# LoganWilliams1/mhm2_kmer_analysis_v2

Measured on AMD Instinct MI355X. Metric: k-mers/sec (kcount stage) at k=21, higher is better.
Workload: dtype u64

## Files before the change

mhm2_kmer_analysis_v2_amd/csrc/kc_bucketed.hpp:

```cpp
#pragma once
#include "kc_kernels.hpp"

namespace kc {

constexpr int WGB = 1024;
constexpr int SUPER_SPAN = 16 * WGB - PRE - POST;
using TileSuper = TileGeo<WGB, SUPER_SPAN>;
static_assert(TileSuper::GPT == 1 && TileSuper::NGROUP == WGB, "one group per thread");
constexpr int PMAX = 1024;
constexpr int GMAX = 512;

template <int NL> struct Rnd {
  static constexpr int RPOS = NL == 1 ? 16 : NL == 2 ? 8 : 4;
  static constexpr int RPOS_READS = NL == 1 ? 8 : NL <= 3 ? 4 : 2;
  static constexpr size_t STAGE = ((size_t)WGB * RPOS + 64) * NL * 8;
  static constexpr size_t STAGE_READS = ((size_t)WGB * RPOS_READS + 64) * NL * 8;
};

struct Geom {
  uint32_t G, P1, P2, S;
  uint32_t log2CH1, log2CH2;
  uint32_t L1MAX, L2MAX;
  uint32_t A1;
  uint32_t A2;
  uint32_t cp;
  uint32_t la, lb;
  uint32_t k2;
  uint32_t own_lo, own_hi;
  uint32_t rec6;
};

struct BucketBufs {
  uint64_t *rec1;
  uint32_t *chain1;
  uint32_t *cnt1;
  uint32_t *used1;
  uint64_t *rec2;
  uint32_t *chain2;
  uint32_t *cnt2;
  uint32_t *base2;
  uint32_t *flag;
  uint64_t *ovf1;
  uint64_t *ovf2;
  uint64_t ovf1_cap, ovf2_cap;
  uint32_t *done1;
  uint32_t *used2;
};

constexpr uint32_t FLAT_MAX = 256;
struct FlatSrc {
  const uint32_t *cnt;
  const uint64_t *at;
  uint32_t F, nbo;
  uint32_t b_lo, b_hi;
};

enum {
  CB_OVF1 = 0, CB_OVF2, CB_FATAL, CB_FLAGGED_RECS, CB_DUMP, CB_ENTRIES, CB_OUT_RESERVED, CB_COUNT = 16
};
enum { FATAL_OVF1 = 1,
       FATAL_ARENA2 = 2,
       FATAL_OVF2 = 4 };


__device__ __forceinline__ uint32_t hash_b1(uint64_t h, const Geom &g) { return (((uint32_t)h & 0xFFFFu) * g.P1) >> 16; }
__device__ __forceinline__ uint32_t hash_b2(uint64_t h, const Geom &g) { return ((((uint32_t)h >> 16) & 0xFFFFu) * g.P2) >> 16; }
__device__ __forceinline__ uint32_t hash_slot(uint64_t h, uint32_t S) {
  return (uint32_t)(h >> 32) & (S - 1u);
}

__device__ __forceinline__ uint64_t cp_mix_rec(uint64_t keyrec, const Geom &g) {
  const uint32_t sh = 64u - g.k2;
  return (kc_feistel_fwd(keyrec >> sh, (int)(g.k2 >> 1)) << sh) | (keyrec & KC_EXT_MASK);
}
__device__ __forceinline__ uint64_t cp_unmix_rec(uint64_t mixrec, const Geom &g) {
  const uint32_t sh = 64u - g.k2;
  return (kc_feistel_inv(mixrec >> sh, (int)(g.k2 >> 1)) << sh) | (mixrec & KC_EXT_MASK);
}
__device__ __forceinline__ uint32_t cp_b1(uint64_t rec, const Geom &g) { return (uint32_t)(rec >> (64u - g.la)); }
__device__ __forceinline__ uint32_t cp_b2(uint64_t rec, const Geom &g) { return (uint32_t)(rec >> (64u - g.la - g.lb)) & (g.P2 - 1u); }
__device__ __forceinline__ uint32_t cp_pack32(uint64_t rec, const Geom &g) {
  const uint32_t rb = g.k2 - g.la - g.lb;
  return (((uint32_t)(rec >> (64u - g.k2)) & ((1u << rb) - 1u)) << 6) | ((uint32_t)rec & (uint32_t)KC_EXT_MASK);
}
__device__ __forceinline__ uint64_t cp_unpack_rec(uint32_t rec32, size_t region, const Geom &g) {
  const uint32_t rb = g.k2 - g.la - g.lb;
  const uint64_t mix = ((uint64_t)region << rb) | (uint64_t)(rec32 >> 6);
  return (kc_feistel_inv(mix, (int)(g.k2 >> 1)) << (64u - g.k2)) | (uint64_t)(rec32 & (uint32_t)KC_EXT_MASK);
}

template <int NL>
__device__ __forceinline__ uint64_t rec_hash(const uint64_t (&rec)[NL]) {
  uint64_t key[NL];
#pragma unroll
  for (int j = 0; j < NL; j++) key[j] = rec[j];
  key[NL - 1] &= ~KC_EXT_MASK;
  return kc_hash<NL>(key);
}

__device__ __forceinline__ void lds_barrier() { asm volatile("s_waitcnt lgkmcnt(0)\n\ts_barrier" ::: "memory"); }

__device__ __forceinline__ int fresh_tid() {
  int t = threadIdx.x;
  asm volatile("" : "+v"(t));
  return t;
}

struct ScanLDS {
  uint32_t wsum[32];
  uint32_t total;
};

__device__ __forceinline__ uint32_t wave_incl_scan(uint32_t v) {
  v += (uint32_t)__builtin_amdgcn_update_dpp(0, (int)v, 0x111, 0xF, 0xF, false);
  v += (uint32_t)__builtin_amdgcn_update_dpp(0, (int)v, 0x112, 0xF, 0xF, false);
  v += (uint32_t)__builtin_amdgcn_update_dpp(0, (int)v, 0x114, 0xF, 0xF, false);
  v += (uint32_t)__builtin_amdgcn_update_dpp(0, (int)v, 0x118, 0xF, 0xF, false);
  v += (uint32_t)__builtin_amdgcn_update_dpp(0, (int)v, 0x142, 0xA, 0xF, false);
  v += (uint32_t)__builtin_amdgcn_update_dpp(0, (int)v, 0x143, 0xC, 0xF, false);
  return v;
}

__device__ __forceinline__ uint32_t block_excl_scan(uint32_t v, ScanLDS &S) {
  static_assert(WGB / 64 <= 16, "the wave totals must fit one row of 16 lanes");
  const int tid = threadIdx.x;
  const int wave = __builtin_amdgcn_readfirstlane(tid >> 6);
  const uint32_t incl = wave_incl_scan(v);
  if (lane_id() == 63) S.wsum[wave] = incl;
  lds_barrier();
  const uint32_t w = (lane_id() < WGB / 64) ? S.wsum[lane_id()] : 0u;
  uint32_t wi = w;
  wi += (uint32_t)__builtin_amdgcn_update_dpp(0, (int)wi, 0x111, 0xF, 0xF, false);
  wi += (uint32_t)__builtin_amdgcn_update_dpp(0, (int)wi, 0x112, 0xF, 0xF, false);
  wi += (uint32_t)__builtin_amdgcn_update_dpp(0, (int)wi, 0x114, 0xF, 0xF, false);
  wi += (uint32_t)__builtin_amdgcn_update_dpp(0, (int)wi, 0x118, 0xF, 0xF, false);
  const uint32_t wave_pre = (uint32_t)__builtin_amdgcn_readlane((int)(wi - w), wave);
  const uint32_t total = (uint32_t)__builtin_amdgcn_readlane((int)wi, WGB / 64 - 1);
  if (tid == 0) S.total = total;
  return incl - v + wave_pre;
}

struct SplitLDS {
  uint32_t hist[2][PMAX + 64];
  uint4 dst[PMAX];
  uint32_t arena_used;
  uint32_t arena_top;
  ScanLDS scan;
};

__device__ __forceinline__ uint32_t hist_rank(SplitLDS &L, int buf, uint32_t b, bool valid) {
  return atomicAdd(&L.hist[buf][valid ? b : (uint32_t)PMAX + lane_id()], 1u);
}

#ifdef KC_STAMPS
#define KC_SPLIT_STAMP(k)                                                                 \
  if (threadIdx.x == 0 && D.stamps) {                                                     \
    const unsigned long long tn_ = __builtin_amdgcn_s_memtime();                          \
    atomicAdd((unsigned long long *)&D.stamps[k], tn_ - *D.tprev);                        \
    *D.tprev = tn_;                                                                       \
  }
#else
#define KC_SPLIT_STAMP(k)
#endif

struct ChainDest {
#ifdef KC_STAMPS
  uint64_t *stamps;
  unsigned long long *tprev;
#endif
  uint64_t *arena;
  uint32_t *chain;
  uint32_t log2CH, LMAX;
  uint32_t arena_cap;
  uint32_t arena_base;
  uint32_t own_lo, own_hi;
};

struct ChainState {
  uint32_t cur;
  uint32_t last;
};

struct RunPlace {
  uint32_t x, y, fit, w;
};
__device__ __forceinline__ RunPlace split_reserve(SplitLDS &L, uint32_t tid, uint32_t v, uint32_t excl, const ChainDest &D, ChainState &st) {
  const uint32_t CHm = (1u << D.log2CH) - 1u;
  const uint32_t base = st.cur;
  uint32_t fit = v;
  const uint64_t room = ((uint64_t)D.LMAX << D.log2CH) - base;
  if ((uint64_t)fit > room) fit = (uint32_t)room;
  const uint32_t have = (base + CHm) >> D.log2CH;
  uint32_t k = ((base + fit + CHm) >> D.log2CH) - have, a = 0;
  if (k) {
    const bool own = tid >= D.own_lo && tid < D.own_hi;
    if (own) {
      a = atomicAdd(&L.arena_used, k);
      const uint32_t left = D.arena_cap - min(D.arena_cap, L.arena_top);
      if (a + k > left) {
        k = a < left ? left - a : 0;
        const uint64_t cap = ((uint64_t)(have + k) << D.log2CH) - base;
        if ((uint64_t)fit > cap) fit = (uint32_t)cap;
      }
    } else {
      const uint32_t t = atomicAdd(&L.arena_top, k);
      const uint32_t left = D.arena_cap - min(D.arena_cap, L.arena_used);
      if (t + k > left) {
        k = 0;
        const uint64_t cap = ((uint64_t)have << D.log2CH) - base;
        if ((uint64_t)fit > cap) fit = (uint32_t)cap;
      } else {
        a = D.arena_cap - t - k;
      }
    }
    uint32_t *ch = D.chain + (size_t)tid * D.LMAX + have;
    for (uint32_t i = 0; i < k; i++) ch[i] = D.arena_base + a + i;
  }
  RunPlace q;
  q.x = ((st.last - D.arena_base - (base >> D.log2CH)) << D.log2CH) + base - excl;
  q.y = ((a - have) << D.log2CH) + base - excl;
  q.fit = fit;
  q.w = (base & CHm) ? min(fit, (CHm + 1u) - (base & CHm)) : 0u;
  if (k) st.last = D.arena_base + a + k - 1;
  st.cur = base + fit;
  return q;
}

template <int NL, int R, int RS = 10, class RecFn>
__device__ __forceinline__ uint32_t split_stage(SplitLDS &L, uint64_t *sorted, uint16_t *sbucket, int buf, uint32_t P, RecFn rec_of,
                                                const uint32_t (&br)[R], const ChainDest &D, ChainState &st) {
  static_assert(R * WGB <= 32768, "positions in the staging must fit 16 bits");
  static_assert(RS == 10 || R * WGB <= 65536, "ranks must fit the bits above RS");
  const int tid = fresh_tid();
  KC_SPLIT_STAMP(1)
  const uint32_t v = ((uint32_t)tid < P) ? L.hist[buf][tid] : 0u;
  const uint32_t excl = block_excl_scan(v, L.scan);
  if ((uint32_t)tid < P) {
    const RunPlace q = split_reserve(L, (uint32_t)tid, v, excl, D, st);
    L.dst[tid] = make_uint4(q.x, q.y, excl | (q.fit << 16), q.w);
    L.hist[buf][tid] = excl;
    L.hist[buf ^ 1][tid] = 0;
  }
  lds_barrier();
  KC_SPLIT_STAMP(2)
  const uint32_t total = L.scan.total;
  constexpr int H = R < 8 ? R : 8;
#pragma unroll
  for (int j0 = 0; j0 < R; j0 += H) {
    uint32_t pos[H];
#pragma unroll
    for (int j = 0; j < H; j++) pos[j] = L.hist[buf][br[j0 + j] & (PMAX - 1)];
#pragma unroll
    for (int j = 0; j < H; j++) {
      const uint32_t bj = br[j0 + j];
      const uint32_t p = bj != ~0u ? pos[j] + (bj >> RS) : (uint32_t)(R * WGB) + lane_id();
      uint64_t r[NL];
      rec_of(j0 + j, r);
#pragma unroll
      for (int w = 0; w < NL; w++) sorted[(size_t)p * NL + w] = r[w];
      if (sbucket) sbucket[p] = (uint16_t)(bj & (PMAX - 1));
    }
  }
  lds_barrier();
  KC_SPLIT_STAMP(3)
  return total;
}

template <int NL, class BucketFn, class OvfFn, class StoreFn>
__device__ __forceinline__ void split_copy_out(SplitLDS &L, const uint64_t *sorted, const uint16_t *sbucket, uint32_t total, const ChainDest &D,
                                               BucketFn bucket_of, OvfFn overflow, StoreFn store) {
  const int tid = fresh_tid();
  constexpr int U = NL == 1 ? 4 : 2;
  const size_t arena0 = (size_t)D.arena_base << D.log2CH;
  for (uint32_t i0 = tid; i0 < total; i0 += U * WGB) {
    uint64_t r[U][NL];
    uint32_t b[U];
    uint4 d[U];
#pragma unroll
    for (int u = 0; u < U; u++) {
      const uint32_t i = i0 + u * WGB;
      const uint32_t ii = i < total ? i : i0;
#pragma unroll
      for (int w = 0; w < NL; w++) r[u][w] = sorted[(size_t)ii * NL + w];
      if (sbucket) b[u] = sbucket[ii];
    }
    if (!sbucket) {
#pragma unroll
      for (int u = 0; u < U; u++) b[u] = bucket_of(r[u]);
    }
#pragma unroll
    for (int u = 0; u < U; u++) d[u] = L.dst[b[u]];
    bool spill = false;
#pragma unroll
    for (int u = 0; u < U; u++) {
      const uint32_t i = i0 + u * WGB;
      const uint32_t j = i - (d[u].z & 0xFFFFu);
      const bool live = i < total, fits = j < (d[u].z >> 16);
      const uint32_t at = (j < d[u].w ? d[u].x : d[u].y) + i;
      if (live && fits) store(arena0 + at, r[u]);
      spill |= live && !fits;
    }
    if (__any(spill)) {
#pragma unroll
      for (int u = 0; u < U; u++) {
        const uint32_t i = i0 + u * WGB;
        if (i < total && i - (d[u].z & 0xFFFFu) >= (d[u].z >> 16)) overflow(b[u], r[u]);
      }
    }
  }
  KC_SPLIT_STAMP(4)
}

template <int NL>
__device__ __forceinline__ void store_words(uint64_t *arena, size_t i, const uint64_t (&r)[NL]) {
#pragma unroll
  for (int w = 0; w < NL; w++) arena[i * NL + w] = r[w];
}

__device__ __forceinline__ ChainState split_load_state(SplitLDS &L, uint32_t P, const uint32_t *cnt, const uint32_t *chain,
                                                       uint32_t LMAX, uint32_t log2CH, uint32_t used, uint32_t top = 0) {
  const int tid = threadIdx.x;
  ChainState st;
  st.cur = 0;
  st.last = 0;
  if ((uint32_t)tid < P) {
    const uint32_t c = cnt ? cnt[tid] : 0u;
    st.cur = c;
    if (c & ((1u << log2CH) - 1u)) st.last = chain[(size_t)tid * LMAX + (c >> log2CH)];
    L.hist[0][tid] = 0;
    L.hist[1][tid] = 0;
  }
  if (tid == 0) {
    L.arena_used = used;
    L.arena_top = top;
  }
  return st;
}

__global__ __launch_bounds__(WGB) void kc_arena_probe_kernel(uint64_t *arena, size_t words_per_wg, uint32_t rounds) {
  uint64_t *mine = arena + (size_t)blockIdx.x * words_per_wg;
  const uint32_t t = threadIdx.x, b = t >> 3, w = t & 7u;
  const size_t chunks = words_per_wg / 512u;
  const size_t hop = chunks > 1024u ? (chunks - 1024u) / 31u : 0u;
  for (uint32_t r = 0; r < rounds; r++) {
    const size_t first = (size_t)((r >> 3) & 31u) * hop;
#pragma unroll
    for (uint32_t j = 0; j < 8; j++) {
      const size_t chunk = first + b + 128u * j;
      const size_t at = chunk * 512u + (size_t)(r & 7u) * 8u + w;
      if (at < words_per_wg) mine[at] = (uint64_t)r;
    }
  }
}

struct L1LDS {
  TileLDS<TileSuper> tile;
  SplitLDS sp;
};

template <int NL>
__device__ __forceinline__ ChainDest l1_dest(const Geom &gm, const BucketBufs &bb, uint32_t g) {
  ChainDest D;
#ifdef KC_STAMPS
  D.stamps = nullptr;
  D.tprev = nullptr;
#endif
  D.arena = bb.rec1 + (((size_t)g * gm.A1) << gm.log2CH1) * NL;
  D.chain = bb.chain1 + (size_t)g * gm.P1 * gm.L1MAX;
  D.log2CH = gm.log2CH1;
  D.LMAX = gm.L1MAX;
  D.arena_cap = gm.A1;
  D.arena_base = 0;
  D.own_lo = gm.own_lo;
  D.own_hi = gm.own_hi;
  return D;
}

__device__ __forceinline__ ChainDest l1_dest6(const Geom &gm, const BucketBufs &bb, uint32_t g) {
  ChainDest D = l1_dest<1>(gm, bb, g);
  D.arena = reinterpret_cast<uint64_t *>(reinterpret_cast<uint8_t *>(bb.rec1) + (((size_t)g * gm.A1) << gm.log2CH1) * 6);
  return D;
}

template <int NL, bool CP>
__device__ __forceinline__ void l1_overflow(const Geom &gm, const BucketBufs &bb, uint64_t *cb, const uint64_t (&r)[NL]) {
  const uint64_t o = atomicAdd((unsigned long long *)&cb[CB_OVF1], 1ULL);
  if (o < bb.ovf1_cap) {
#pragma unroll
    for (int w = 0; w < NL; w++) bb.ovf1[o * NL + w] = (CP && w == 0) ? cp_unmix_rec(r[w], gm) : r[w];
  } else {
    atomicOr((unsigned long long *)&cb[CB_FATAL], (unsigned long long)FATAL_OVF1);
  }
}

template <int KT, int RPOS, bool SH, class TL>
__device__ __forceinline__ void cp_run_fixed(const TL &L, int lp0, bool active, const Geom &gm, const ExtractArgs &a, uint32_t (&lo)[RPOS],
                                             uint32_t (&bk)[RPOS]) {
  const int K = KT ? KT : (int)a.k;
  const int NB = RPOS + K + 1;
  static_assert(RPOS + KT + 1 <= 32 && RPOS % 8 == 0 && PRE % 8 == 0, "the window must fit one word and never start word-aligned");
  const uint64_t *W = reinterpret_cast<const uint64_t *>(L.codes);
  const uint32_t *OK = reinterpret_cast<const uint32_t *>(L.ok);
  const int p = lp0 - 1, q = p >> 5, s = p & 31;
  const uint64_t w0 = W[q], w1 = W[q + 1];
  const uint32_t ok0 = OK[q], ok1 = OK[q + 1], g0 = L.gap[q], g1 = L.gap[q + 1];
  const uint64_t Wn = (w0 << (2 * s)) | (w1 >> (64 - 2 * s));
  const uint32_t nok = ~__builtin_amdgcn_alignbit(ok1, ok0, (uint32_t)s);
  const uint32_t gapw = __builtin_amdgcn_alignbit(g1, g0, (uint32_t)s);
  const uint64_t Rn = kc_rc_word(Wn) << (64 - 2 * NB);
  const uint64_t MID = ((1ULL << (2 * K)) - 1ULL) << 2;
  const uint32_t MK = (1u << K) - 1u;
#pragma unroll
  for (int j = 0; j < RPOS; j++) {
    const uint64_t x = Wn >> (64 - 2 * (j + K + 2)), y = Rn >> (64 - 2 * (RPOS - 1 - j + K + 2));
    const uint64_t CMP = (K & 1) ? (MID | 3ULL) : MID;
    const bool swap = (y & CMP) < (x & CMP);
    const uint64_t sel = swap ? y : x;
    const uint32_t na = (nok >> j) & 1u, nb = (nok >> (j + K + 1)) & 1u;
    const uint32_t le = ((uint32_t)(sel >> (2 * K + 2)) & 3u) | ((swap ? nb : na) << 2);
    const uint32_t re = ((uint32_t)sel & 3u) | ((swap ? na : nb) << 2);
    uint32_t Lh = (uint32_t)(sel >> (K + 2)) & MK, Rh = (uint32_t)(sel >> 2) & MK;
    bool valid = active && ((gapw >> (j + 1)) & ((1u << (K + 1)) - 1u)) == 0u;
    if (SH) {
      uint64_t key[1] = {(((uint64_t)Lh << K) | Rh) << (64 - 2 * K)};
      const uint32_t owner = a.reference_owner ? 0u : kc_owner_of_hash(kc_hash<1>(key), a.rank_n);
      if (a.reference_owner) {
        uint64_t rk[1];
        kc_revcomp<1>(key, K, rk);
        valid = valid && kc_reference_owner<1>(key, rk, K, a.rank_n) == a.rank_me;
      } else {
        valid = valid && owner == a.rank_me;
      }
    }
    Lh ^= kc_feistel_f(Rh, 0, K);
    Rh ^= kc_feistel_f(Lh, 1, K);
    Lh ^= kc_feistel_f(Rh, 2, K);
    const uint64_t mix = ((uint64_t)Lh << K) | Rh;
    lo[j] = (uint32_t)mix;
    bk[j] = valid ? ((uint32_t)(mix >> (2 * K - gm.la)) | (le << 10) | (re << 13)) : ~0u;
  }
}

template <int K, int RPOS, class TL>
__device__ __forceinline__ uint32_t cut_run_fixed(const TL &L, int lp0, bool active, uint64_t (&rec)[RPOS], uint64_t (&h)[RPOS]) {
  constexpr int NB = RPOS + K + 1;
  static_assert(NB <= 32 && RPOS % 8 == 0 && PRE % 8 == 0, "the window must fit one word and never start word-aligned");
  const uint64_t *W = reinterpret_cast<const uint64_t *>(L.codes);
  const uint32_t *OK = reinterpret_cast<const uint32_t *>(L.ok);
  const int p = lp0 - 1, q = p >> 5, s = p & 31;
  const uint64_t w0 = W[q], w1 = W[q + 1];
  const uint32_t ok0 = OK[q], ok1 = OK[q + 1], g0 = L.gap[q], g1 = L.gap[q + 1];
  const uint64_t Wn = (w0 << (2 * s)) | (w1 >> (64 - 2 * s));
  const uint32_t nok = ~__builtin_amdgcn_alignbit(ok1, ok0, (uint32_t)s);
  const uint32_t gapw = __builtin_amdgcn_alignbit(g1, g0, (uint32_t)s);
  const uint64_t Rn = kc_rc_word(Wn) << (64 - 2 * NB);
  constexpr uint64_t MID = ((1ULL << (2 * K)) - 1ULL) << 2;
  constexpr uint64_t CMP = (K & 1) ? (MID | 3ULL) : MID;
  uint32_t okm = 0;
#pragma unroll
  for (int j = 0; j < RPOS; j++) {
    const uint64_t x = Wn >> (64 - 2 * (j + K + 2)), y = Rn >> (64 - 2 * (RPOS - 1 - j + K + 2));
    const bool swap = (y & CMP) < (x & CMP);
    const uint64_t sel = swap ? y : x;
    const uint32_t na = (nok >> j) & 1u, nb = (nok >> (j + K + 1)) & 1u;
    const uint32_t le = ((uint32_t)(sel >> (2 * K + 2)) & 3u) | ((swap ? nb : na) << 2);
    const uint32_t re = ((uint32_t)sel & 3u) | ((swap ? na : nb) << 2);
    const uint64_t key = (sel >> 2) << (64 - 2 * K);
    const uint64_t kk[1] = {key};
    h[j] = kc_hash<1>(kk);
    rec[j] = key | (uint64_t)((le & 4u) ? 4u : le) | ((uint64_t)((re & 4u) ? 4u : re) << 3);
    const bool valid = active && ((gapw >> (j + 1)) & ((1u << (K + 1)) - 1u)) == 0u;
    okm |= valid ? (1u << j) : 0u;
  }
  return okm;
}

template <int NL, int FMT, bool CP, bool SH>
__global__ __launch_bounds__(WGB) void kc_l1_reads_kernel(ExtractArgs a, Geom gm, BucketBufs bb, uint64_t nsuper, uint32_t rot,
                                                          uint64_t *ctrs, uint64_t *cb) {
  extern __shared__ __align__(16) uint8_t smem[];
  L1LDS &L = *reinterpret_cast<L1LDS *>(smem);
  uint64_t *sorted = reinterpret_cast<uint64_t *>(smem + ((sizeof(L1LDS) + 15) & ~size_t(15)));
  uint16_t *sbucket = CP ? nullptr : reinterpret_cast<uint16_t *>(smem + ((sizeof(L1LDS) + 15) & ~size_t(15)) + Rnd<NL>::STAGE_READS);
  constexpr int RPOS = Rnd<NL>::RPOS_READS;
  const int tid = threadIdx.x;
  const uint32_t g = (blockIdx.x + rot) % gm.G, P1 = gm.P1;
  ChainDest D = l1_dest<NL>(gm, bb, g);
#ifdef KC_STAMPS
  unsigned long long tprev_ = __builtin_amdgcn_s_memtime();
  D.stamps = cb + 8;
  D.tprev = &tprev_;
#endif
  ChainState cst = split_load_state(L.sp, P1, bb.cnt1 + (size_t)g * P1, D.chain, D.LMAX, D.log2CH, bb.used1[g], bb.used1[gm.G + g]);
  __syncthreads();
  uint32_t n_ins = 0;
  int buf = 0;
  TileRaw<TileSuper> raw;
  auto first_of = [&](uint64_t st) -> uint64_t { return (FMT != FMT_SEQBLOCK && st < nsuper) ? a.tile_first[st] : 0; };
  tile_prefetch<FMT, TileSuper>(raw, a, a.pos0 + (int64_t)blockIdx.x * SUPER_SPAN, tid, first_of(blockIdx.x), blockIdx.x < nsuper);
  uint64_t next_first = first_of((uint64_t)blockIdx.x + gridDim.x);
  constexpr int RUNS = SUPER_SPAN / RPOS;
  static_assert(SUPER_SPAN % RPOS == 0, "runs must tile the span");
  constexpr int NROUND = (RUNS + WGB - 1) / WGB;
  for (int64_t it = -1;; it++) {
    const uint64_t st = (uint64_t)blockIdx.x + (uint64_t)(it < 0 ? 0 : it) * gridDim.x;
    const bool work = it >= 0;
    if (work && st >= nsuper) break;
#pragma unroll 1
    for (int round = 0; round < NROUND; round++) {
      uint64_t rec[RPOS][NL];
      uint32_t br[RPOS];
      uint32_t total = 0;
      if (work) {
      const int run_id = round * WGB + tid;
      const bool active = run_id < RUNS;
      const int lp0 = PRE + (active ? run_id : 0) * RPOS;
      KmerRun<NL> run;
      run_begin<NL>(run, L.tile, lp0, a.k);
#pragma unroll
      for (int j = 0; j < RPOS; j++) {
        uint64_t h = 0;
        uint32_t owner = 0;
        bool valid = run_kmer<NL, !CP>(run, j, lp0, a.k, rec[j], h, SH ? a.rank_n : 1u, SH ? a.reference_owner : 0u, SH ? &owner : nullptr) && active;
        if (SH) {
          if (CP && !a.reference_owner) {
            uint64_t key[NL];
#pragma unroll
            for (int w = 0; w < NL; w++) key[w] = rec[j][w];
            key[NL - 1] &= ~KC_EXT_MASK;
            owner = kc_owner_of_hash(kc_hash<NL>(key), a.rank_n);
          }
          valid = valid && owner == a.rank_me;
        }
        if (CP) rec[j][0] = cp_mix_rec(rec[j][0], gm);
        br[j] = valid ? (CP ? cp_b1(rec[j][0], gm) : hash_b1(h, gm)) : ~0u;
        if (j + 1 < RPOS) run_advance<NL>(run, j, lp0, a.k);
      }
#pragma unroll
      for (int j = 0; j < RPOS; j++) {
        const bool valid = br[j] != ~0u;
        const uint32_t rank = hist_rank(L.sp, buf, br[j] & (PMAX - 1), valid);
        br[j] = valid ? (br[j] | (rank << 10)) : ~0u;
        n_ins += valid ? 1u : 0u;
      }
      KC_SPLIT_STAMP(0)
      lds_barrier();
      total = split_stage<NL, RPOS>(
          L.sp, sorted, sbucket, buf, P1,
          [&](int j, uint64_t (&o)[NL]) {
#pragma unroll
            for (int w = 0; w < NL; w++) o[w] = rec[j][w];
          },
          br, D, cst);
      }
      if (round == NROUND - 1) {
        const uint64_t nst = work ? st + gridDim.x : st;
        tile_encode<FMT, TileSuper>(L.tile, raw, a, a.pos0 + (int64_t)nst * SUPER_SPAN, ctrs, tid, nst < nsuper);
        tile_prefetch<FMT, TileSuper>(raw, a, a.pos0 + (int64_t)(nst + gridDim.x) * SUPER_SPAN, tid, next_first, nst + gridDim.x < nsuper);
        next_first = first_of(nst + 2 * (uint64_t)gridDim.x);
        KC_SPLIT_STAMP(5)
      }
      if (work) {
        split_copy_out<NL>(
            L.sp, sorted, sbucket, total, D, [&](const uint64_t (&r)[NL]) { return cp_b1(r[0], gm); },
            [&](uint32_t, const uint64_t (&r)[NL]) { l1_overflow<NL, CP>(gm, bb, cb, r); },
            [&](size_t i, const uint64_t (&r)[NL]) { store_words<NL>(D.arena, i, r); });
        buf ^= 1;
      }
    }
  }
  if ((uint32_t)tid < P1) bb.cnt1[(size_t)g * P1 + tid] = cst.cur;
  if (tid == 0) {
    bb.used1[g] = min(L.sp.arena_used, gm.A1);
    bb.used1[gm.G + g] = min(L.sp.arena_top, gm.A1);
  }
  for (int o = 32; o > 0; o >>= 1) n_ins += __shfl_down(n_ins, o);
  if (lane_id() == 0 && n_ins) atomicAdd((unsigned long long *)&ctrs[CTR_INSERTED], (unsigned long long)n_ins);
}

constexpr int R16 = 16;
constexpr uint32_t ST16_MAIN = (uint32_t)WGB * R16 + PMAX;
constexpr uint32_t ST16_SLOTS = ST16_MAIN + 64;
static_assert(SUPER_SPAN % R16 == 0 && SUPER_SPAN / R16 <= WGB, "one run of sixteen positions per thread covers the super-tile");
static_assert(ST16_MAIN < 65536, "staging positions fit 16 bits");
constexpr size_t l1x16_lds_bytes() { return ((sizeof(L1LDS) + 15) & ~size_t(15)) + (size_t)ST16_SLOTS * 6; }

template <class MidFn>
__device__ __forceinline__ uint32_t split_stage_pairs(SplitLDS &L, uint32_t *slo, uint16_t *sbk, int buf, uint32_t P, const uint32_t (&lo)[R16],
                                                      const uint32_t (&br)[R16], const ChainDest &D, ChainState &st, MidFn mid) {
  const int tid = fresh_tid();
  KC_SPLIT_STAMP(1)
  const uint32_t v = ((uint32_t)tid < P) ? L.hist[buf][tid] : 0u;
  const uint32_t excl = block_excl_scan((v + 1u) & ~1u, L.scan);
// ... 31 lines not shown
    }
    uint4 d;
    d.x = ((st.last - D.arena_base - (base >> D.log2CH)) << D.log2CH) + base - excl;
    d.y = ((a - have) << D.log2CH) + base - excl;
    d.z = excl | (v << 16);
    d.w = fit | (((base & CHm) ? min(fit, (CHm + 1u) - (base & CHm)) : 0u) << 16);
    L.dst[tid] = d;
    if (k) st.last = D.arena_base + a + k - 1;
    st.cur = base + fit;
    L.hist[buf][tid] = excl;
    L.hist[buf ^ 1][tid] = 0;
  }
  lds_barrier();
  KC_SPLIT_STAMP(2)
  const uint32_t total = L.scan.total;
#pragma unroll
  for (int j0 = 0; j0 < R16; j0 += 8) {
    uint32_t pos[8];
#pragma unroll
    for (int j = 0; j < 8; j++) pos[j] = L.hist[buf][br[j0 + j] & (PMAX - 1)];
#pragma unroll
    for (int j = 0; j < 8; j++) {
      const uint32_t bj = br[j0 + j];
      const uint32_t p = bj != ~0u ? pos[j] + (bj >> 16) : ST16_MAIN + lane_id();
      slo[p] = lo[j0 + j];
      sbk[p] = (uint16_t)bj;
    }
  }
  mid();
  lds_barrier();
  KC_SPLIT_STAMP(3)
  return total;
}

struct __attribute__((packed, aligned(2))) Rec6Pair {
  uint32_t w0, w1, w2;
};
struct __attribute__((packed, aligned(2))) Rec6 {
  uint32_t lo;
  uint16_t bk;
};
static_assert(sizeof(Rec6Pair) == 12 && sizeof(Rec6) == 6, "six bytes a record");

template <class OvfFn>
__device__ __forceinline__ void split_copy_out_pairs(SplitLDS &L, const uint32_t *slo, const uint16_t *sbk, uint32_t total, const ChainDest &D,
                                                     const Geom &gm, OvfFn overflow) {
  const int tid = fresh_tid();
  constexpr int U = 2;
  uint8_t *const arena0 = reinterpret_cast<uint8_t *>(D.arena) + ((size_t)D.arena_base << D.log2CH) * 6;
  const uint32_t shb = 64u - gm.la, shl = 64u - gm.k2;
  for (uint32_t i0 = 2u * (uint32_t)tid; i0 < total; i0 += 2u * U * WGB) {
    uint64_t lo2[U];
    uint32_t bk2[U];
    uint4 d[U];
#pragma unroll
    for (int u = 0; u < U; u++) {
      const uint32_t i = i0 + 2u * (uint32_t)u * WGB;
      const uint32_t ii = i < total ? i : i0;
      lo2[u] = *reinterpret_cast<const uint64_t *>(slo + ii);
      bk2[u] = *reinterpret_cast<const uint32_t *>(sbk + ii);
    }
#pragma unroll
    for (int u = 0; u < U; u++) d[u] = L.dst[bk2[u] & (PMAX - 1)];
    bool odd = false;
#pragma unroll
    for (int u = 0; u < U; u++) {
      const uint32_t i = i0 + 2u * (uint32_t)u * WGB;
      const uint32_t j = i - (d[u].z & 0xFFFFu), v = d[u].z >> 16, fit = d[u].w & 0xFFFFu, wold = d[u].w >> 16;
      const bool live = i < total;
      const bool f0 = live && j < fit, real1 = live && j + 1u < v, f1 = real1 && j + 1u < fit;
      const uint32_t at0 = (j < wold ? d[u].x : d[u].y) + i, at1 = (j + 1u < wold ? d[u].x : d[u].y) + i + 1u;
      const bool pair = f0 && f1 && at1 == at0 + 1u;
      if (pair) {
        const uint32_t l1 = (uint32_t)(lo2[u] >> 32);
        Rec6Pair r;
        r.w0 = (uint32_t)lo2[u];
        r.w1 = (bk2[u] & 0xFFFFu) | (l1 << 16);
        r.w2 = (l1 >> 16) | (bk2[u] & 0xFFFF0000u);
        *reinterpret_cast<Rec6Pair *>(arena0 + (size_t)at0 * 6) = r;
      } else if (f0) {
        Rec6 r;
        r.lo = (uint32_t)lo2[u];
        r.bk = (uint16_t)bk2[u];
        *reinterpret_cast<Rec6 *>(arena0 + (size_t)at0 * 6) = r;
      }
      odd |= (real1 && !pair) || (live && !f0);
    }
    if (__any(odd)) {
#pragma unroll
      for (int u = 0; u < U; u++) {
        const uint32_t i = i0 + 2u * (uint32_t)u * WGB;
        if (i >= total) continue;
        const uint32_t j = i - (d[u].z & 0xFFFFu), v = d[u].z >> 16, fit = d[u].w & 0xFFFFu, wold = d[u].w >> 16;
        const uint32_t at0 = (j < wold ? d[u].x : d[u].y) + i, at1 = (j + 1u < wold ? d[u].x : d[u].y) + i + 1u;
        const uint32_t l0 = (uint32_t)lo2[u], l1 = (uint32_t)(lo2[u] >> 32);
        const uint64_t bh = (uint64_t)(bk2[u] & (PMAX - 1)) << shb;
        const uint64_t ra = bh | ((uint64_t)l0 << shl) | (uint64_t)((bk2[u] >> 10) & 63u);
        const uint64_t rb = bh | ((uint64_t)l1 << shl) | (uint64_t)(bk2[u] >> 26);
        const bool f0 = j < fit, real1 = j + 1u < v, f1 = real1 && j + 1u < fit;
        if (!f0) overflow(ra);
        if (real1 && !(f0 && f1 && at1 == at0 + 1u)) {
          if (f1) {
            Rec6 r;
            r.lo = l1;
            r.bk = (uint16_t)(bk2[u] >> 16);
            *reinterpret_cast<Rec6 *>(arena0 + (size_t)at1 * 6) = r;
          } else {
            overflow(rb);
          }
        }
      }
    }
  }
  KC_SPLIT_STAMP(4)
}

template <int FMT, bool SH, int KK>
__global__ __launch_bounds__(WGB) void kc_l1_reads16_kernel(ExtractArgs a, Geom gm, BucketBufs bb, uint64_t nsuper, uint32_t rot, uint64_t *ctrs,
                                                            uint64_t *cb) {
  extern __shared__ __align__(16) uint8_t smem[];
  L1LDS &L = *reinterpret_cast<L1LDS *>(smem);
  uint32_t *slo = reinterpret_cast<uint32_t *>(smem + ((sizeof(L1LDS) + 15) & ~size_t(15)));
  uint16_t *sbk = reinterpret_cast<uint16_t *>(slo + ST16_SLOTS);
  const int tid = threadIdx.x;
  const uint32_t g = (blockIdx.x + rot) % gm.G, P1 = gm.P1;
  ChainDest D = l1_dest6(gm, bb, g);
#ifdef KC_STAMPS
  unsigned long long tprev_ = __builtin_amdgcn_s_memtime();
  D.stamps = cb + 8;
  D.tprev = &tprev_;
#endif
  ChainState cst = split_load_state(L.sp, P1, bb.cnt1 + (size_t)g * P1, D.chain, D.LMAX, D.log2CH, bb.used1[g], bb.used1[gm.G + g]);
  __syncthreads();
  uint32_t n_ins = 0;
  int buf = 0;
  TileRaw<TileSuper> raw;
  auto first_of = [&](uint64_t st) -> uint64_t { return (FMT != FMT_SEQBLOCK && st < nsuper) ? a.tile_first[st] : 0; };
  tile_prefetch<FMT, TileSuper>(raw, a, a.pos0 + (int64_t)blockIdx.x * SUPER_SPAN, tid, first_of(blockIdx.x), blockIdx.x < nsuper);
  uint64_t next_first = first_of((uint64_t)blockIdx.x + gridDim.x);
  constexpr int RUNS = SUPER_SPAN / R16;
  {
    const int ft = fresh_tid();
    tile_encode<FMT, TileSuper>(L.tile, raw, a, a.pos0 + (int64_t)blockIdx.x * SUPER_SPAN, ctrs, ft, blockIdx.x < nsuper);
    tile_prefetch<FMT, TileSuper>(raw, a, a.pos0 + (int64_t)((uint64_t)blockIdx.x + gridDim.x) * SUPER_SPAN, ft, next_first,
                                  (uint64_t)blockIdx.x + gridDim.x < nsuper);
    next_first = first_of((uint64_t)blockIdx.x + 2 * (uint64_t)gridDim.x);
  }
  for (uint64_t st = blockIdx.x; st < nsuper; st += gridDim.x) {
    uint32_t lo[R16], br[R16];
    const bool active = tid < RUNS;
    const int lp0 = PRE + (active ? tid : 0) * R16;
    {
      uint32_t l8[8], b8[8];
      cp_run_fixed<KK, 8, SH>(L.tile, lp0, active, gm, a, l8, b8);
#pragma unroll
      for (int j = 0; j < 8; j++) {
        lo[j] = l8[j];
        br[j] = b8[j];
      }
      cp_run_fixed<KK, 8, SH>(L.tile, lp0 + 8, active, gm, a, l8, b8);
#pragma unroll
      for (int j = 0; j < 8; j++) {
        lo[8 + j] = l8[j];
        br[8 + j] = b8[j];
      }
    }
#pragma unroll
    for (int j = 0; j < R16; j++) {
      const bool valid = br[j] != ~0u;
      const uint32_t rank = hist_rank(L.sp, buf, br[j] & (PMAX - 1), valid);
      br[j] = valid ? (br[j] | (rank << 16)) : ~0u;
      n_ins += valid ? 1u : 0u;
    }
    KC_SPLIT_STAMP(0)
    lds_barrier();
    const int ft = fresh_tid();
    const uint64_t nst = st + gridDim.x;
    tile_encode_clear<TileSuper>(L.tile, raw, ft);
    const uint32_t total = split_stage_pairs(L.sp, slo, sbk, buf, P1, lo, br, D, cst, [&]() {
      tile_encode_fill<FMT, TileSuper>(L.tile, raw, a, a.pos0 + (int64_t)nst * SUPER_SPAN, ctrs, ft, nst < nsuper);
      tile_prefetch<FMT, TileSuper>(raw, a, a.pos0 + (int64_t)(nst + gridDim.x) * SUPER_SPAN, ft, next_first, nst + gridDim.x < nsuper);
      next_first = first_of(nst + 2 * (uint64_t)gridDim.x);
    });
    split_copy_out_pairs(L.sp, slo, sbk, total, D, gm, [&](uint64_t r) {
      const uint64_t rr[1] = {r};
      l1_overflow<1, true>(gm, bb, cb, rr);
    });
    buf ^= 1;
  }
  if ((uint32_t)tid < P1) bb.cnt1[(size_t)g * P1 + tid] = cst.cur;
  if (tid == 0) {
    bb.used1[g] = min(L.sp.arena_used, gm.A1);
    bb.used1[gm.G + g] = min(L.sp.arena_top, gm.A1);
  }
  for (int o = 32; o > 0; o >>= 1) n_ins += __shfl_down(n_ins, o);
  if (lane_id() == 0 && n_ins) atomicAdd((unsigned long long *)&ctrs[CTR_INSERTED], (unsigned long long)n_ins);
}

template <int NL, int R>
__device__ __forceinline__ void split_round_flat(SplitLDS &L, int buf, uint32_t P, const uint64_t (&rec)[R][NL], const uint32_t (&br)[R],
                                                 uint64_t *records, uint64_t seg_cap, uint64_t *cursors, uint64_t *overflow_flag) {
  const int tid = threadIdx.x;
  if ((uint32_t)tid < P) {
    const uint32_t v = L.hist[buf][tid];
    uint64_t base = 0;
    if (v) base = atomicAdd((unsigned long long *)&cursors[tid], (unsigned long long)v);
    const uint64_t room = base < seg_cap ? seg_cap - base : 0;
    uint4 d;
    d.x = (uint32_t)base;
    d.y = (uint32_t)(base >> 32);
    d.z = (uint64_t)v <= room ? v : (uint32_t)room;
    d.w = 0;
    L.dst[tid] = d;
    L.hist[buf ^ 1][tid] = 0;
  }
  lds_barrier();
#pragma unroll
  for (int j = 0; j < R; j++) {
    if (br[j] != ~0u) {
      const uint32_t b = br[j] & (PMAX - 1), rank = br[j] >> 10;
      const uint4 d = L.dst[b];
      if (rank < d.z) {
        uint64_t *o = records + ((uint64_t)b * seg_cap + (((uint64_t)d.y << 32) | d.x) + rank) * NL;
#pragma unroll
        for (int w = 0; w < NL; w++) o[w] = rec[j][w];
      } else {
        *overflow_flag = 1;
      }
    }
  }
}

template <int NL, int FMT>
__global__ __launch_bounds__(WGB) void kc_bin_reads_kernel(ExtractArgs a, uint64_t nsuper, uint64_t *ctrs) {
  extern __shared__ __align__(16) uint8_t smem[];
  L1LDS &L = *reinterpret_cast<L1LDS *>(smem);
  constexpr int RPOS = Rnd<NL>::RPOS_READS;
  const int tid = threadIdx.x;
  const uint32_t P = a.rank_n;
  if ((uint32_t)tid < PMAX) {
    L.sp.hist[0][tid] = 0;
    L.sp.hist[1][tid] = 0;
  }
  __syncthreads();
  int buf = 0;
  TileRaw<TileSuper> raw;
  auto first_of = [&](uint64_t st) -> uint64_t { return (FMT != FMT_SEQBLOCK && st < nsuper) ? a.tile_first[st] : 0; };
  tile_prefetch<FMT, TileSuper>(raw, a, a.pos0 + (int64_t)blockIdx.x * SUPER_SPAN, tid, first_of(blockIdx.x), blockIdx.x < nsuper);
  uint64_t next_first = first_of((uint64_t)blockIdx.x + gridDim.x);
  constexpr int RUNS = SUPER_SPAN / RPOS;
  static_assert(SUPER_SPAN % RPOS == 0, "runs must tile the span");
  for (uint64_t st = blockIdx.x; st < nsuper; st += gridDim.x) {
    const int64_t T0 = a.pos0 + (int64_t)st * SUPER_SPAN;
    tile_encode<FMT, TileSuper>(L.tile, raw, a, T0, ctrs, tid, true);
    {
      const uint64_t nst = st + gridDim.x;
      tile_prefetch<FMT, TileSuper>(raw, a, a.pos0 + (int64_t)nst * SUPER_SPAN, tid, next_first, nst < nsuper);
      next_first = first_of(nst + gridDim.x);
    }
#pragma unroll 1
    for (int round = 0; round < (RUNS + WGB - 1) / WGB; round++) {
      uint64_t rec[RPOS][NL];
      uint32_t br[RPOS];
      const int run_id = round * WGB + tid;
      const bool active = run_id < RUNS;
      const int lp0 = PRE + (active ? run_id : 0) * RPOS;
      bool fixed21 = false;
      uint32_t okm = 0;
      uint64_t hh[RPOS];
      if constexpr (NL == 1 && RPOS == 8) {
        fixed21 = a.k == 21 && !a.reference_owner;
        if (fixed21) okm = cut_run_fixed<21, 8>(L.tile, lp0, active, reinterpret_cast<uint64_t (&)[RPOS]>(rec), hh);
      }
      KmerRun<NL> run;
      if (!fixed21) run_begin<NL>(run, L.tile, lp0, a.k);
#pragma unroll
      for (int j = 0; j < RPOS; j++) {
        uint64_t h = 0;
        uint32_t owner = 0;
        bool valid;
        if (fixed21) {
          valid = (okm >> j) & 1u;
          owner = kc_owner_of_hash(hh[j], P);
        } else {
          valid = run_kmer<NL>(run, j, lp0, a.k, rec[j], h, P, a.reference_owner, &owner) && active;
          if (j + 1 < RPOS) run_advance<NL>(run, j, lp0, a.k);
        }
        br[j] = ~0u;
        const uint32_t b = P > 1 ? owner : 0u;
        if (P <= 16) {
          for (uint32_t d = 0; d < P; d++) {
            const bool mine = valid && b == d;
            const uint64_t m = __ballot(mine);
            if (m) {
              const int leader = __ffsll((long long)m) - 1;
              uint32_t base = 0;
              if ((int)lane_id() == leader) base = atomicAdd(&L.sp.hist[buf][d], (uint32_t)__popcll(m));
              base = __shfl(base, leader);
              if (mine) br[j] = d | ((base + (uint32_t)__popcll(m & ((1ULL << lane_id()) - 1ULL))) << 10);
            }
          }
        } else if (valid) {
          const uint32_t rank = atomicAdd(&L.sp.hist[buf][b], 1u);
          br[j] = b | (rank << 10);
        }
      }
      lds_barrier();
      split_round_flat<NL, RPOS>(L.sp, buf, P, rec, br, a.records, a.seg_capacity, ctrs + CTR_BIN0, ctrs + CTR_OVERFLOW);
      buf ^= 1;
    }
  }
}

struct L1RLDS {
  SplitLDS sp;
};

template <int NL, bool CP>
__global__ __launch_bounds__(WGB) void kc_l1_records_kernel(const uint64_t *recs, uint64_t n, Geom gm, BucketBufs bb, uint32_t rot,
                                                            uint64_t *ctrs, uint64_t *cb) {
  extern __shared__ __align__(16) uint8_t smem[];
  L1RLDS &L = *reinterpret_cast<L1RLDS *>(smem);
  uint64_t *sorted = reinterpret_cast<uint64_t *>(smem + ((sizeof(L1RLDS) + 15) & ~size_t(15)));
  constexpr int RPOS = Rnd<NL>::RPOS;
  const int tid = threadIdx.x;
  const uint32_t g = (blockIdx.x + rot) % gm.G, P1 = gm.P1;
// ... 1428 lines not shown
```

mhm2_kmer_analysis_v2_amd/csrc/kc_common.hpp:

```cpp
#pragma once
#include <stdint.h>

#if defined(__HIPCC__)
#include <hip/hip_runtime.h>
#define KC_HD __host__ __device__ __forceinline__
#else
#define KC_HD static inline
#endif

#define KC_MAX_LONGS 4
#define KC_QUAL_CUTOFF 20
#define KC_EXT_NONE 4u
#define KC_EXT_BITS 6
#define KC_EXT_MASK 0x3FULL
#define KC_COUNT_MAX 65535u

KC_HD uint32_t kc_base_code(uint32_t c) {
  uint32_t b = (c >> 1) & 3u;
  return b ^ (b >> 1);
}

KC_HD bool kc_is_acgt(uint32_t c) {
  uint32_t u = c & 0xDFu;
  return u == 'A' || u == 'C' || u == 'G' || u == 'T';
}

KC_HD bool kc_is_base_char(uint32_t c) {
  uint32_t u = c & 0xDFu;
  return u == 'A' || u == 'C' || u == 'G' || u == 'T' || u == 'N';
}

KC_HD uint64_t kc_rc_word(uint64_t v) {
#if defined(__HIP_DEVICE_COMPILE__)
  v = __brevll(v);
  v = ((v >> 1) & 0x5555555555555555ULL) | ((v & 0x5555555555555555ULL) << 1);
#else
  v = ((v >> 2) & 0x3333333333333333ULL) | ((v & 0x3333333333333333ULL) << 2);
  v = ((v >> 4) & 0x0F0F0F0F0F0F0F0FULL) | ((v & 0x0F0F0F0F0F0F0F0FULL) << 4);
  v = __builtin_bswap64(v);
#endif
  return ~v;
}

KC_HD uint64_t kc_word_mask(int k, int j) {
  int nb = k - 32 * j;
  if (nb >= 32) return ~0ULL;
  if (nb <= 0) return 0ULL;
  return ~(~0ULL >> (2 * nb));
}

template <int NL>
KC_HD void kc_revcomp(const uint64_t (&w)[NL], int k, uint64_t (&out)[NL]) {
  const int ll = (k + 31) / 32;
  uint64_t t[NL];
#pragma unroll
  for (int i = 0; i < NL; i++) {
    uint64_t v = 0;
#pragma unroll
    for (int j = 0; j < NL; j++)
      if (j == ll - 1 - i) v = kc_rc_word(w[j]);
    t[i] = v;
  }
  const int sh = 64 * ll - 2 * k;
  if (sh) {
#pragma unroll
    for (int j = 0; j < NL; j++) {
      uint64_t nxt = (j + 1 < NL) ? t[j + 1] : 0ULL;
      t[j] = (t[j] << sh) | (nxt >> (64 - sh));
    }
  }
#pragma unroll
  for (int j = 0; j < NL; j++) out[j] = (j < ll) ? t[j] : 0ULL;
}

template <int NL>
KC_HD bool kc_less(const uint64_t (&a)[NL], const uint64_t (&b)[NL]) {
#pragma unroll
  for (int j = 0; j < NL; j++) {
    if (a[j] < b[j]) return true;
    if (a[j] > b[j]) return false;
  }
  return false;
}

KC_HD void kc_mum32(uint32_t &a, uint32_t &b, uint32_t ca, uint32_t cb) {
  const uint64_t c = (uint64_t)(a ^ ca) * (uint64_t)(b ^ cb);
  a = (uint32_t)c;
  b = (uint32_t)(c >> 32);
}

template <int NL>
KC_HD uint64_t kc_hash(const uint64_t (&key)[NL]) {
  uint32_t a = 0x9E3779B9u, b = 0x85EBCA6Bu;
#pragma unroll
  for (int j = 0; j < NL; j++) {
    a ^= (uint32_t)key[j];
    b ^= (uint32_t)(key[j] >> 32);
    kc_mum32(a, b, 0x53c5ca59u, 0x74743c1bu);
  }
  uint32_t a2 = a, b2 = b;
  kc_mum32(a, b, 0x53c5ca59u, 0x74743c1bu);
  kc_mum32(a2, b2, 0xa0761d65u, 0xe7037ed1u);
  return ((uint64_t)(a2 ^ b2) << 32) | (uint64_t)(a ^ b);
}

KC_HD uint32_t kc_feistel_f(uint32_t x, int i, int k) {
  const uint32_t C[3] = {0x9E3779u, 0x85EBCBu, 0xC2B2AFu}, D[3] = {0x7F4A7Cu, 0x165667u, 0x3C6EF3u};
#if defined(__HIP_DEVICE_COMPILE__)
  return (__umul24(x, C[i]) + D[i]) >> (32 - k);
#else
  return (x * C[i] + D[i]) >> (32 - k);
#endif
}
KC_HD uint64_t kc_feistel_fwd(uint64_t v, int k) {
  uint32_t L = (uint32_t)(v >> k), R = (uint32_t)v & ((1u << k) - 1u);
  L ^= kc_feistel_f(R, 0, k);
  R ^= kc_feistel_f(L, 1, k);
  L ^= kc_feistel_f(R, 2, k);
  return ((uint64_t)L << k) | R;
}
KC_HD uint64_t kc_feistel_inv(uint64_t m, int k) {
  uint32_t L = (uint32_t)(m >> k), R = (uint32_t)m & ((1u << k) - 1u);
  L ^= kc_feistel_f(R, 2, k);
  R ^= kc_feistel_f(L, 1, k);
  L ^= kc_feistel_f(R, 0, k);
  return ((uint64_t)L << k) | R;
}
constexpr int KC_COMPACT_MAX_K = 23;

KC_HD uint32_t kc_owner_of_hash(uint64_t h, uint32_t rank_n) {
  return (uint32_t)(((h >> 32) * (uint64_t)rank_n) >> 32);
}

KC_HD uint64_t kc_quick_hash(uint64_t v) {
  v = v * 3935559000370003845ULL + 2691343689449507681ULL;
  v ^= v >> 21;
  v ^= v << 37;
  v ^= v >> 4;
  v *= 4768777513237032717ULL;
  v ^= v << 20;
  v ^= v >> 41;
  v ^= v << 5;
  return v;
}

KC_HD int kc_minimizer_len(int k) {
  int m = k * 2 / 3 + 1;
  if (m < 15) m = 15;
  if (m > 27) m = 27;
  return m < k ? m : k;
}

template <int NL>
KC_HD uint64_t kc_mmer_at(const uint64_t (&w)[NL], int i, int m) {
  const int l = i >> 5, sh = 2 * (i & 31);
  uint64_t hi = 0, lo = 0;
#pragma unroll
  for (int j = 0; j < NL; j++) {
    if (j == l) hi = w[j];
    if (j == l + 1) lo = w[j];
  }
  const uint64_t t = sh ? ((hi << sh) | (lo >> (64 - sh))) : hi;
  return t & (~0ULL << (64 - 2 * m));
}

template <int NL>
KC_HD uint32_t kc_reference_owner(const uint64_t (&f)[NL], const uint64_t (&r)[NL], int k, uint32_t rank_n) {
  const int m = kc_minimizer_len(k), ncand = k - m + 1;
  uint64_t best = 0;
  for (int i = 0; i < ncand; i++) {
    const uint64_t a = kc_mmer_at<NL>(f, i, m), b = kc_mmer_at<NL>(r, ncand - 1 - i, m);
    const uint64_t least = a < b ? a : b;
    if (least > best) best = least;
  }
  return (uint32_t)(kc_quick_hash(best) % (uint64_t)rank_n);
}

#define KC_SYNTH_MAX_GENOMES 1024

struct kc_synth_table {
  uint64_t seed;
  uint32_t num_genomes;
  uint32_t read_len;
  uint64_t err_thr;
  uint64_t lowq_thr;
  uint64_t n_thr;
  uint64_t genome_len[KC_SYNTH_MAX_GENOMES];
  uint64_t genome_seed[KC_SYNTH_MAX_GENOMES];
  uint64_t cum[KC_SYNTH_MAX_GENOMES];
};

KC_HD uint64_t kc_splitmix(uint64_t x) {
  x += 0x9E3779B97F4A7C15ULL;
  x = (x ^ (x >> 30)) * 0xBF58476D1CE4E5B9ULL;
  x = (x ^ (x >> 27)) * 0x94D049BB133111EBULL;
  return x ^ (x >> 31);
}

KC_HD uint32_t kc_genome_base(uint64_t gseed, uint64_t pos) { return (uint32_t)(kc_splitmix(gseed + pos * 0xD1342543DE82EF95ULL) >> 62); }

KC_HD void kc_synth_base(const kc_synth_table *t, uint64_t rstate, uint32_t g, uint64_t start, bool rev, uint32_t i,
                         uint8_t *base, uint8_t *qual) {
  const uint32_t L = t->read_len;
  uint64_t pos = rev ? start + (L - 1 - i) : start + i;
  uint32_t b = kc_genome_base(t->genome_seed[g], pos);
  if (rev) b = 3u - b;
  uint64_t u = kc_splitmix(rstate + 0x632BE59BD9B4E019ULL * (uint64_t)(i + 1));
  uint8_t q = 'I';
  if (u < t->err_thr) {
    b = (b + 1u + (uint32_t)((u >> 7) % 3u)) & 3u;
    q = '#';
  } else if (u < t->lowq_thr) {
    q = '#';
  }
  uint8_t c = (uint8_t)("ACGT"[b]);
  if (t->n_thr) {
    uint64_t u2 = kc_splitmix(u ^ 0xA5A5A5A5A5A5A5A5ULL);
    if (u2 < t->n_thr) {
      c = 'N';
      q = '#';
    }
  }
  *base = c;
  *qual = q;
}

KC_HD void kc_synth_read_header(const kc_synth_table *t, uint64_t r, uint64_t *rstate, uint32_t *g, uint64_t *start,
                                bool *rev) {
  uint64_t s = kc_splitmix(t->seed ^ (r * 0x9E3779B97F4A7C15ULL));
  uint64_t u1 = kc_splitmix(s + 1), u2 = kc_splitmix(s + 2), u3 = kc_splitmix(s + 3);
  uint32_t lo = 0, hi = t->num_genomes - 1;
  while (lo < hi) {
    uint32_t mid = (lo + hi) >> 1;
    if (u1 <= t->cum[mid]) hi = mid; else lo = mid + 1;
  }
  *g = lo;
  uint64_t span = t->genome_len[lo] - t->read_len + 1;
  *start = u2 % span;
  *rev = (u3 >> 63) != 0;
  *rstate = s;
}
```

Measured before the change: 100.0 billion.

## Rewrite canonical-pass k-mer extraction with bitwise validity masks and branchless bucket packing

Reworks the per-position inner loop of cp_run_fixed. Validity comes from a gap mask precomputed once per 8-position run by a log-step OR cascade, and the canonical comparison works on left-aligned words. The extension bits are assembled with precomputed spread nibble masks and shifts held in VGPRs via an asm barrier. The histogram rank step drops its valid branch by clamping invalid buckets into per-lane dummy slots, and the insert count is returned from the extraction via popcount. All of this cuts scalar/vector ALU work in a compute-bound kcount stage, at the cost of more intricate bit manipulation and a hard requirement that RPOS is 8.

New measurement: 102.1 billion (median of 6 runs). +2.0%, better.

```diff
diff --git a/mhm2_kmer_analysis_v2_amd/csrc/kc_bucketed.hpp b/mhm2_kmer_analysis_v2_amd/csrc/kc_bucketed.hpp
--- a/mhm2_kmer_analysis_v2_amd/csrc/kc_bucketed.hpp
+++ b/mhm2_kmer_analysis_v2_amd/csrc/kc_bucketed.hpp
@@ -150,6 +150,11 @@
 
 __device__ __forceinline__ uint32_t hist_rank(SplitLDS &L, int buf, uint32_t b, bool valid) {
   return atomicAdd(&L.hist[buf][valid ? b : (uint32_t)PMAX + lane_id()], 1u);
+}
+
+__device__ __forceinline__ uint32_t hist_rank_bk(SplitLDS &L, int buf, uint32_t bk) {
+  static_assert(PMAX == 1024, "the bucket is the low ten bits of bk");
+  return atomicAdd(&L.hist[buf][min(bk & ~0xFC00u, (uint32_t)PMAX + lane_id())], 1u);
 }
 
 #ifdef KC_STAMPS
@@ -394,11 +399,11 @@
 }
 
 template <int KT, int RPOS, bool SH, class TL>
-__device__ __forceinline__ void cp_run_fixed(const TL &L, int lp0, bool active, const Geom &gm, const ExtractArgs &a, uint32_t (&lo)[RPOS],
-                                             uint32_t (&bk)[RPOS]) {
+__device__ __forceinline__ uint32_t cp_run_fixed(const TL &L, int lp0, bool active, const Geom &gm, const ExtractArgs &a,
+                                                 uint32_t (&lo)[RPOS], uint32_t (&bk)[RPOS]) {
   const int K = KT ? KT : (int)a.k;
   const int NB = RPOS + K + 1;
-  static_assert(RPOS + KT + 1 <= 32 && RPOS % 8 == 0 && PRE % 8 == 0, "the window must fit one word and never start word-aligned");
+  static_assert(RPOS + KT + 1 <= 32 && RPOS == 8 && PRE % 8 == 0, "the window must fit one word and never start word-aligned");
   const uint64_t *W = reinterpret_cast<const uint64_t *>(L.codes);
   const uint32_t *OK = reinterpret_cast<const uint32_t *>(L.ok);
   const int p = lp0 - 1, q = p >> 5, s = p & 31;
@@ -408,21 +413,37 @@
   const uint32_t nok = ~__builtin_amdgcn_alignbit(ok1, ok0, (uint32_t)s);
   const uint32_t gapw = __builtin_amdgcn_alignbit(g1, g0, (uint32_t)s);
   const uint64_t Rn = kc_rc_word(Wn) << (64 - 2 * NB);
-  const uint64_t MID = ((1ULL << (2 * K)) - 1ULL) << 2;
+  const uint64_t KM = ~0ULL << (64 - 2 * K);
   const uint32_t MK = (1u << K) - 1u;
+  uint32_t bad = gapw >> 1;
+#pragma unroll
+  for (int c = 1; c < K + 1;) {
+    const int d = c < K + 1 - c ? c : K + 1 - c;
+    bad |= bad >> d;
+    c += d;
+  }
+  bad = active ? bad : ~0u;
+  auto spread4 = [](uint32_t v) {
+    v &= 0xFFu;
+    v = (v | (v << 12)) & 0x000F000Fu;
+    v = (v | (v << 6)) & 0x03030303u;
+    return (v | (v << 3)) & 0x11111111u;
+  };
+  const uint32_t na4 = spread4(nok), nb4 = spread4(nok >> (K + 1));
+  const uint32_t Qf = na4 | (nb4 << 3), Qr = nb4 | (na4 << 3);
+  const uint32_t vLh = kc_vreg(32 - K), vb = kc_vreg((uint32_t)K - gm.la), v3 = kc_vreg(3u);
+  const int NSH = 62 - 2 * K, NW = NSH >= 32 ? 32 : 0, NP = NSH - NW;
+  const uint32_t vE = kc_vreg((uint32_t)(NP - 10));
+  uint32_t n = 0;
 #pragma unroll
   for (int j = 0; j < RPOS; j++) {
-    const uint64_t x = Wn >> (64 - 2 * (j + K + 2)), y = Rn >> (64 - 2 * (RPOS - 1 - j + K + 2));
-    const uint64_t CMP = (K & 1) ? (MID | 3ULL) : MID;
-    const bool swap = (y & CMP) < (x & CMP);
-    const uint64_t sel = swap ? y : x;
-    const uint32_t na = (nok >> j) & 1u, nb = (nok >> (j + K + 1)) & 1u;
-    const uint32_t le = ((uint32_t)(sel >> (2 * K + 2)) & 3u) | ((swap ? nb : na) << 2);
-    const uint32_t re = ((uint32_t)sel & 3u) | ((swap ? na : nb) << 2);
-    uint32_t Lh = (uint32_t)(sel >> (K + 2)) & MK, Rh = (uint32_t)(sel >> 2) & MK;
-    bool valid = active && ((gapw >> (j + 1)) & ((1u << (K + 1)) - 1u)) == 0u;
+    const uint64_t X = Wn << (2 * (j + 1)), Y = Rn << (2 * (RPOS - j));
+    const bool swap = (K & 1) ? Y < X : (Y & KM) < (X & KM);
+    const uint64_t sel = swap ? Y : X;
+    uint32_t Lh = (uint32_t)(sel >> 32) >> vLh, Rh = (uint32_t)(sel >> (64 - 2 * K)) & MK;
+    bool valid = !((bad >> j) & 1u);
     if (SH) {
-      uint64_t key[1] = {(((uint64_t)Lh << K) | Rh) << (64 - 2 * K)};
+      uint64_t key[1] = {sel & KM};
       const uint32_t owner = a.reference_owner ? 0u : kc_owner_of_hash(kc_hash<1>(key), a.rank_n);
       if (a.reference_owner) {
         uint64_t rk[1];
@@ -432,13 +453,27 @@
         valid = valid && owner == a.rank_me;
       }
     }
-    Lh ^= kc_feistel_f(Rh, 0, K);
-    Rh ^= kc_feistel_f(Lh, 1, K);
-    Lh ^= kc_feistel_f(Rh, 2, K);
-    const uint64_t mix = ((uint64_t)Lh << K) | Rh;
-    lo[j] = (uint32_t)mix;
-    bk[j] = valid ? ((uint32_t)(mix >> (2 * K - gm.la)) | (le << 10) | (re << 13)) : ~0u;
-  }
+    Lh ^= kc_feistel_m(Rh, 0) >> vLh;
+    Rh ^= kc_feistel_m(Lh, 1) >> vLh;
+    Lh ^= kc_feistel_m(Rh, 2) >> vLh;
+    lo[j] = kc_vreg((Lh << K) | Rh);
+    const uint32_t b = KT >= 10 ? Lh >> vb : (uint32_t)((((uint64_t)Lh << K) | Rh) >> (2 * K - gm.la));
+    const uint32_t sw = (uint32_t)(sel >> NW), ow = ~(sw ^ (uint32_t)(X >> NW) ^ (uint32_t)(Y >> NW));
+    const uint32_t qs = swap ? Qr : Qf;
+    uint32_t e;
+    if (KT && NP >= 10 && NP <= 26) {
+      const uint32_t M1 = 3u << NP, MQ = 9u << (NP + 2);
+      const uint32_t qj = 4 * j <= NP + 2 ? qs << (NP + 2 - 4 * j) : qs >> (4 * j - NP - 2);
+      e = (ow & M1) | ((sw << v3) & ~M1);
+      e = (qj & MQ) | (e & ~MQ);
+      e = (e >> vE) & 0xFC00u;
+    } else {
+      e = (((ow >> NP) & 3u) | (((sw >> NP) & 3u) << 3) | (((qs >> (4 * j)) & 9u) << 2)) << 10;
+    }
+    bk[j] = SH ? (valid ? b | e : ~0u) : (b | e) | (uint32_t)((int32_t)(bad << (31 - j)) >> 31);
+    if (SH) n += valid ? 1u : 0u;
+  }
+  return SH ? n : (uint32_t)__builtin_popcount(~bad & ((1u << RPOS) - 1u));
 }
 
 template <int K, int RPOS, class TL>
@@ -776,13 +811,13 @@
     const int lp0 = PRE + (active ? tid : 0) * R16;
     {
       uint32_t l8[8], b8[8];
-      cp_run_fixed<KK, 8, SH>(L.tile, lp0, active, gm, a, l8, b8);
+      n_ins += cp_run_fixed<KK, 8, SH>(L.tile, lp0, active, gm, a, l8, b8);
 #pragma unroll
       for (int j = 0; j < 8; j++) {
         lo[j] = l8[j];
         br[j] = b8[j];
       }
-      cp_run_fixed<KK, 8, SH>(L.tile, lp0 + 8, active, gm, a, l8, b8);
+      n_ins += cp_run_fixed<KK, 8, SH>(L.tile, lp0 + 8, active, gm, a, l8, b8);
 #pragma unroll
       for (int j = 0; j < 8; j++) {
         lo[8 + j] = l8[j];
@@ -790,12 +825,7 @@
       }
     }
 #pragma unroll
-    for (int j = 0; j < R16; j++) {
-      const bool valid = br[j] != ~0u;
-      const uint32_t rank = hist_rank(L.sp, buf, br[j] & (PMAX - 1), valid);
-      br[j] = valid ? (br[j] | (rank << 16)) : ~0u;
-      n_ins += valid ? 1u : 0u;
-    }
+    for (int j = 0; j < R16; j++) br[j] |= hist_rank_bk(L.sp, buf, br[j]) << 16;
     KC_SPLIT_STAMP(0)
     lds_barrier();
     const int ft = fresh_tid();
diff --git a/mhm2_kmer_analysis_v2_amd/csrc/kc_common.hpp b/mhm2_kmer_analysis_v2_amd/csrc/kc_common.hpp
--- a/mhm2_kmer_analysis_v2_amd/csrc/kc_common.hpp
+++ b/mhm2_kmer_analysis_v2_amd/csrc/kc_common.hpp
@@ -104,14 +104,22 @@
   return ((uint64_t)(a2 ^ b2) << 32) | (uint64_t)(a ^ b);
 }
 
-KC_HD uint32_t kc_feistel_f(uint32_t x, int i, int k) {
+KC_HD uint32_t kc_vreg(uint32_t v) {
+#if defined(__HIP_DEVICE_COMPILE__)
+  asm volatile("" : "+v"(v));
+#endif
+  return v;
+}
+
+KC_HD uint32_t kc_feistel_m(uint32_t x, int i) {
   const uint32_t C[3] = {0x9E3779u, 0x85EBCBu, 0xC2B2AFu}, D[3] = {0x7F4A7Cu, 0x165667u, 0x3C6EF3u};
 #if defined(__HIP_DEVICE_COMPILE__)
-  return (__umul24(x, C[i]) + D[i]) >> (32 - k);
+  return __umul24(x, C[i]) + D[i];
 #else
-  return (x * C[i] + D[i]) >> (32 - k);
-#endif
-}
+  return x * C[i] + D[i];
+#endif
+}
+KC_HD uint32_t kc_feistel_f(uint32_t x, int i, int k) { return kc_feistel_m(x, i) >> (32 - k); }
 KC_HD uint64_t kc_feistel_fwd(uint64_t v, int k) {
   uint32_t L = (uint32_t)(v >> k), R = (uint32_t)v & ((1u << k) - 1u);
   L ^= kc_feistel_f(R, 0, k);
```
